# prs-eth/ResDepth

Measured on AMD Instinct MI355X. Metric: DSM tiles/sec fwd+bwd (256x256, 3-ch, depth-5 U-Net), higher is better.
Workload: dtype f32

## Files before the change

### resdepth_amd/csrc/rd_elementwise.hip

```cpp
#include <stdlib.h>

#include "rd_common.h"
#include "rd_mfma_dev.h"

namespace rd {

static inline int grid_cap(long g, int cap) {
    if (g > cap) g = cap;
    if (g < 1) g = 1;
    return (int)g;
}

__device__ __forceinline__ float act_fn(float y, float slope) { return y > 0.f ? y : y * slope; }
__device__ __forceinline__ float act_grad(float y, float slope) { return y > 0.f ? 1.f : slope; }

template <int K>
__device__ __forceinline__ void reduce_rows(double (&vals)[K], double* red, int t, int CQ, int RP, bool active) {
#pragma unroll
    for (int k = 0; k < K; ++k) red[k * 256 + t] = active ? vals[k] : 0.0;
    __syncthreads();
    if (t < CQ) {
#pragma unroll
        for (int k = 0; k < K; ++k) {
            double s = 0.0;
// ... 156 lines not shown
            const float v0 = partial[(long)b * 2 * C + col], v1 = partial[(long)(b + 32) * 2 * C + col];
            const float v2 = partial[(long)(b + 64) * 2 * C + col], v3 = partial[(long)(b + 96) * 2 * C + col];
            sacc += ((double)v0 + (double)v1) + ((double)v2 + (double)v3);
        }
        for (; b < nb; b += 32) sacc += (double)partial[(long)b * 2 * C + col];
    }
    red[t] = sacc;
    __syncthreads();
    if (t == 0 && blockIdx.x == 0 && nbt) *nbt += 1;
    if (t < 4 && c < C) {
        double su = 0.0, sq = 0.0;
#pragma unroll
        for (int sl = 0; sl < 32; ++sl) {
            su += red[sl * 8 + t];
            sq += red[sl * 8 + 4 + t];
        }
        const double m = su / count;
        double var = sq / count - m * m;
        if (var < 0.0) var = 0.0;
        mean[c] = (float)m;
        invstd[c] = (float)(1.0 / sqrt(var + (double)eps));
        if (rmean) rmean[c] = (1.f - momentum) * rmean[c] + momentum * (float)m;
        if (rvar) {
            const double unb = count > 1.0 ? var * count / (count - 1.0) : var;
            rvar[c] = (1.f - momentum) * rvar[c] + momentum * (float)unb;
        }
    }
}

__global__ __launch_bounds__(256) void bn_bwd_stats_finalize_kernel(const float* __restrict__ pa, int ra,
                                                                    const float* __restrict__ pb, int rb, int C,
                                                                    double* __restrict__ sums, float* __restrict__ dgamma,
                                                                    float* __restrict__ dbeta, float* __restrict__ dextra) {
    __shared__ double wred[4][4];
    const int t = threadIdx.x, lane = t & 63, wave = t >> 6, CQ = C >> 2;
    const int sidx = blockIdx.x / CQ, cq = blockIdx.x - sidx * CQ;
    const long col = (long)sidx * C + cq * 4, stride = 4L * C;
    double a0 = 0.0, a1 = 0.0, a2 = 0.0, a3 = 0.0;
    for (int src = 0; src < 2; ++src) {
        const float* part = src ? pb : pa;
        const int nb = src ? rb : ra;
        if (!part) continue;
        int b = t;
        for (; b + 768 < nb; b += 1024) {
            const float4 v0 = *reinterpret_cast<const float4*>(part + (long)b * stride + col);
            const float4 v1 = *reinterpret_cast<const float4*>(part + (long)(b + 256) * stride + col);
            const float4 v2 = *reinterpret_cast<const float4*>(part + (long)(b + 512) * stride + col);
            const float4 v3 = *reinterpret_cast<const float4*>(part + (long)(b + 768) * stride + col);
            a0 += ((double)v0.x + (double)v1.x) + ((double)v2.x + (double)v3.x);
            a1 += ((double)v0.y + (double)v1.y) + ((double)v2.y + (double)v3.y);
            a2 += ((double)v0.z + (double)v1.z) + ((double)v2.z + (double)v3.z);
            a3 += ((double)v0.w + (double)v1.w) + ((double)v2.w + (double)v3.w);
        }
        for (; b < nb; b += 256) {
            const float4 v = *reinterpret_cast<const float4*>(part + (long)b * stride + col);
            a0 += v.x; a1 += v.y; a2 += v.z; a3 += v.w;
        }
    }
#pragma unroll
    for (int o = 1; o < 64; o <<= 1) {
        a0 += __shfl_xor(a0, o);
        a1 += __shfl_xor(a1, o);
        a2 += __shfl_xor(a2, o);
        a3 += __shfl_xor(a3, o);
    }
    if (lane == 0) {
        wred[wave][0] = a0; wred[wave][1] = a1; wred[wave][2] = a2; wred[wave][3] = a3;
    }
    __syncthreads();
    if (t < 4) {
        const double r = ((wred[0][t] + wred[1][t]) + wred[2][t]) + wred[3][t];
        const int c = cq * 4 + t;
        sums[col + t] = r;
        if (sidx == 0 && dbeta) dbeta[c] = (float)r;
        if (sidx == 1 && dgamma) dgamma[c] = (float)r;
        if (sidx == 2 && dextra) dextra[c] = (float)r;
    }
}

__global__ __launch_bounds__(512) void bn_reduce_finalize_quad_kernel(const float* __restrict__ partial, int nb, int C, double count,
                                                                      float eps, float momentum, float* __restrict__ mean,
                                                                      float* __restrict__ invstd, float* __restrict__ rmean,
                                                                      float* __restrict__ rvar, int64_t* nbt) {
    __shared__ double red[512][4];
    const int t = threadIdx.x, kind = t & 1, slice = t >> 1, cq = blockIdx.x;
    const float* base = partial + (long)kind * C + cq * 4;
    const long stride = 2L * C;
    double a0 = 0.0, a1 = 0.0, a2 = 0.0, a3 = 0.0;
    int b = slice;
    for (; b + 7 * 256 < nb; b += 8 * 256) {
        float4 v[8];
#pragma unroll
        for (int k = 0; k < 8; ++k) v[k] = *reinterpret_cast<const float4*>(base + (long)(b + 256 * k) * stride);
#pragma unroll
        for (int k = 0; k < 8; ++k) {
            a0 += v[k].x; a1 += v[k].y; a2 += v[k].z; a3 += v[k].w;
        }
    }
    for (; b < nb; b += 256) {
        const float4 v = *reinterpret_cast<const float4*>(base + (long)b * stride);
        a0 += v.x; a1 += v.y; a2 += v.z; a3 += v.w;
    }
    red[t][0] = a0; red[t][1] = a1; red[t][2] = a2; red[t][3] = a3;
    __syncthreads();
    for (int sl = 128; sl >= 1; sl >>= 1) {
        if (slice < sl) {
#pragma unroll
            for (int k = 0; k < 4; ++k) red[t][k] += red[t + 2 * sl][k];
        }
        __syncthreads();
    }
    if (t == 0 && blockIdx.x == 0 && nbt) *nbt += 1;
    if (t < 4) {
        const int c = cq * 4 + t;
        const double su = red[0][t], sq = red[1][t];
        const double m = su / count;
        double var = sq / count - m * m;
        if (var < 0.0) var = 0.0;
        mean[c] = (float)m;
        invstd[c] = (float)(1.0 / sqrt(var + (double)eps));
        if (rmean) rmean[c] = (1.f - momentum) * rmean[c] + momentum * (float)m;
        if (rvar) {
            const double unb = count > 1.0 ? var * count / (count - 1.0) : var;
            rvar[c] = (1.f - momentum) * rvar[c] + momentum * (float)unb;
        }
    }
}

int bn_reduce_finalize(const float* partial, int nb, int c, double count, float eps, float momentum, float* mean, float* invstd,
                       float* rmean, float* rvar, int64_t* nbt, hipStream_t s) {
    if (c % 4 == 0)
        RD_LAUNCH(bn_reduce_finalize_quad_kernel, dim3(c / 4), dim3(512), 0, s, partial, nb, c, count, eps, momentum, mean,
                           invstd, rmean, rvar, nbt);
    else
        RD_LAUNCH(bn_reduce_finalize_kernel, dim3(cdiv(c, 4)), dim3(256), 0, s, partial, nb, c, count, eps, momentum, mean,
                           invstd, rmean, rvar, nbt);
    RD_LAUNCH_CHECK("bn_reduce_finalize");
    return RD_OK;
}

__global__ void bn_eval_stats_kernel(const float* __restrict__ rmean, const float* __restrict__ rvar, float eps,
                                     float* __restrict__ mean, float* __restrict__ invstd, int C) {
    const int c = blockIdx.x * blockDim.x + threadIdx.x;
    if (c >= C) return;
    mean[c] = rmean[c];
    invstd[c] = 1.f / sqrtf(rvar[c] + eps);
}

template <bool POOL>
__global__ __launch_bounds__(256) void bn_act_pool_fwd_kernel(const float* __restrict__ z, const float* __restrict__ mean,
                                                              const float* __restrict__ invstd,
                                                              const float* __restrict__ gamma,
                                                              const float* __restrict__ beta, float slope_val,
                                                              const float* __restrict__ slope_dev,
                                                              float* __restrict__ a, float* __restrict__ pooled,
                                                              uint8_t* __restrict__ idx, float* __restrict__ zpool, long rows,
                                                              int H, int W, int C, int CQ, unsigned* a_amax, unsigned* p_amax) {
    const float slope = slope_dev ? slope_dev[0] : slope_val;
    const long total = rows * CQ;
    float amx = 0.f, pmx = 0.f;
    long e0, e1;
    block_range(total, blockIdx.x, gridDim.x, blockDim.x, e0, e1);
    for (long e = e0 + threadIdx.x; e < e1; e += blockDim.x) {
        const int cq = (int)(e % CQ);
        const long row = e / CQ;
        const float4 mu = *reinterpret_cast<const float4*>(mean + cq * 4);
        const float4 is = *reinterpret_cast<const float4*>(invstd + cq * 4);
        const float4 ga = *reinterpret_cast<const float4*>(gamma + cq * 4);
        const float4 be = *reinterpret_cast<const float4*>(beta + cq * 4);
        const float sc[4] = {is.x * ga.x, is.y * ga.y, is.z * ga.z, is.w * ga.w};
        const float sh[4] = {be.x - mu.x * sc[0], be.y - mu.y * sc[1], be.z - mu.z * sc[2], be.w - mu.w * sc[3]};
        if (!POOL) {
            const float4 x = ld_nt4(z + row * C + cq * 4);
            float4 y;
            y.x = act_fn(fmaf(x.x, sc[0], sh[0]), slope);
            y.y = act_fn(fmaf(x.y, sc[1], sh[1]), slope);
            y.z = act_fn(fmaf(x.z, sc[2], sh[2]), slope);
            y.w = act_fn(fmaf(x.w, sc[3], sh[3]), slope);
            *reinterpret_cast<float4*>(a + row * C + cq * 4) = y;
            amx = amax_acc(amax_acc(amax_acc(amax_acc(amx, y.x), y.y), y.z), y.w);
        } else {
            const int W2 = W >> 1, H2 = H >> 1;
            const int j = (int)(row % W2);
            const int i = (int)((row / W2) % H2);
            const long img = row / ((long)W2 * H2);
            const long base = (img * H + 2 * i) * W + 2 * j;
            float m[4], zm[4] = {0.f, 0.f, 0.f, 0.f};
            int mi[4] = {0, 0, 0, 0};
#pragma unroll
            for (int k = 0; k < 4; ++k) {
                const long pix = base + (k >> 1) * W + (k & 1);
                const float4 x = ld_nt4(z + pix * C + cq * 4);
                const float xv[4] = {x.x, x.y, x.z, x.w};
                float y[4];
                y[0] = act_fn(fmaf(x.x, sc[0], sh[0]), slope);
                y[1] = act_fn(fmaf(x.y, sc[1], sh[1]), slope);
                y[2] = act_fn(fmaf(x.z, sc[2], sh[2]), slope);
                y[3] = act_fn(fmaf(x.w, sc[3], sh[3]), slope);
                if (a) *reinterpret_cast<float4*>(a + pix * C + cq * 4) = make_float4(y[0], y[1], y[2], y[3]);
#pragma unroll
                for (int q = 0; q < 4; ++q) {
                    if (k == 0 || y[q] > m[q] || y[q] != y[q]) {
                        m[q] = y[q];
                        mi[q] = k;
                        zm[q] = xv[q];
                    }
                }
            }
            *reinterpret_cast<float4*>(pooled + row * C + cq * 4) = make_float4(m[0], m[1], m[2], m[3]);
            pmx = amax_acc(amax_acc(amax_acc(amax_acc(pmx, m[0]), m[1]), m[2]), m[3]);
            if (zpool) st_nt4(zpool + row * C + cq * 4, make_float4(zm[0], zm[1], zm[2], zm[3]));
            st_nt_u8x4(idx + row * C + cq * 4,
                       make_uchar4((unsigned char)mi[0], (unsigned char)mi[1], (unsigned char)mi[2], (unsigned char)mi[3]));
        }
// ... 1153 lines not shown
                       mean, invstd, running_mean, running_var, nbt, c);
    RD_LAUNCH_CHECK("bn_finalize");
    return RD_OK;
}

int rd_bn_eval_stats(const float* running_mean, const float* running_var, float eps, float* mean, float* invstd, int c,
                     rd_stream_t s) {
    RD_REQUIRE(running_mean && running_var && mean && invstd && c > 0, "rd_bn_eval_stats: bad arguments");
    RD_LAUNCH(bn_eval_stats_kernel, dim3(cdiv(c, 256)), dim3(256), 0, (hipStream_t)s, running_mean,
                       running_var, eps, mean, invstd, c);
    RD_LAUNCH_CHECK("bn_eval_stats");
    return RD_OK;
}

int rd_bn_act_pool_fwd(const float* z, const float* mean, const float* invstd, const float* gamma, const float* beta,
                       float slope, const float* slope_dev, float* a, float* pooled, uint8_t* idx, float* zpool, int n, int h,
                       int w, int c, rd_stream_t s) {
    RD_REQUIRE(z && mean && invstd && gamma && beta && (a || pooled), "rd_bn_act_pool_fwd: null pointer");
    RD_REQUIRE(c % 4 == 0 && c > 0, "rd_bn_act_pool_fwd: C must be a multiple of 4 (got %d)", c);
    const QuantArgs qa = quant_take();
    const int CQ = c / 4;
    const long pixels = (long)n * h * w;
    if (pooled) {
        RD_REQUIRE(idx && h % 2 == 0 && w % 2 == 0, "rd_bn_act_pool_fwd: pooling needs idx and even H, W");
        const long rows = pixels / 4;
        ProfScope ps((hipStream_t)s, "bn_act_pool_fwd", 0,
                     4.0 * pixels * c * (a ? 2.25 : 1.25) + 0.25 * pixels * c + (zpool ? 1.0 * pixels * c : 0.0));
        RD_LAUNCH((bn_act_pool_fwd_kernel<true>), dim3(grid_cap((rows * CQ + 255) / 256, 8192)), dim3(256), 0,
                           (hipStream_t)s, z, mean, invstd, gamma, beta, slope, slope_dev, a, pooled, idx, zpool, rows, h, w, c,
                           CQ, (unsigned*)nullptr, qa.out2);
    } else {
        ProfScope ps((hipStream_t)s, "bn_act_fwd", 0, 8.0 * pixels * c);
        RD_LAUNCH((bn_act_pool_fwd_kernel<false>), dim3(grid_cap((pixels * CQ + 255) / 256, 8192)), dim3(256),
                           0, (hipStream_t)s, z, mean, invstd, gamma, beta, slope, slope_dev, a, (float*)nullptr,
                           (uint8_t*)nullptr, (float*)nullptr, pixels, h, w, c, CQ, qa.out, (unsigned*)nullptr);
    }
    RD_LAUNCH_CHECK("bn_act_pool_fwd");
    return RD_OK;
}

size_t rd_bn_act_bwd_ws_bytes(int n, int h, int w, int c) {
    RowPlan pl;
    if (!plan_rows((long)n * h * w, c, &pl)) return 0;
    return (size_t)pl.nb * 4 * c * sizeof(double);
}

int rd_bn_act_bwd_reduce(const float* z, const float* mean, const float* invstd, const float* gamma, const float* beta,
                         float slope, const float* slope_dev, const float* g_full, const float* g_pool,
                         const uint8_t* idx, double* sums, float* dgamma, float* dbeta, float* dextra, int n, int h, int w, int c,
                         void* ws, size_t ws_bytes, rd_stream_t s) {
    RD_REQUIRE(z && mean && invstd && gamma && beta && sums, "rd_bn_act_bwd_reduce: null pointer");
    RD_REQUIRE(g_full || g_pool, "rd_bn_act_bwd_reduce: no gradient source");
    RD_REQUIRE(!g_pool || idx, "rd_bn_act_bwd_reduce: g_pool needs idx");
    const bool pool = g_pool != nullptr;
    const long pixels = (long)n * h * w;
    const long rows = pool ? pixels / 4 : pixels;
    RowPlan pl;
    RD_REQUIRE(plan_rows(rows, c, &pl), "rd_bn_act_bwd_reduce: C must be a multiple of 4 and <= 1024 (got %d)", c);
    size_t need = (size_t)pl.nb * 4 * c * sizeof(double);
    if (const size_t q = rd_bn_act_bwd_ws_bytes(n, h, w, c); q > need) need = q;
    if (!ws || ws_bytes < need) {
        set_error("rd_bn_act_bwd_reduce: workspace too small (%zu < %zu)", ws_bytes, need);
        return RD_ERR_WS;
    }
    ProfScope ps((hipStream_t)s, "bn_act_bwd_reduce", 0, 4.0 * pixels * c * (1 + (g_full ? 1 : 0) + (pool ? 0.3 : 0)));
    if (pool)
        RD_LAUNCH((bn_act_bwd_kernel<true, false>), dim3(pl.nb), dim3(256), 0, (hipStream_t)s, z, mean, invstd,
                           gamma, beta, slope, slope_dev, g_full, g_pool, idx, (double*)ws, (const double*)nullptr, 1.0, 1,
                           (float*)nullptr, rows, h, w, c, pl.CQ, pl.RP, pl.rows_per_block, (unsigned*)nullptr);
    else
        RD_LAUNCH((bn_act_bwd_kernel<false, false>), dim3(pl.nb), dim3(256), 0, (hipStream_t)s, z, mean,
                           invstd, gamma, beta, slope, slope_dev, g_full, g_pool, idx, (double*)ws, (const double*)nullptr, 1.0, 1,
                           (float*)nullptr, rows, h, w, c, pl.CQ, pl.RP, pl.rows_per_block, (unsigned*)nullptr);
    RD_LAUNCH(partial_reduce_kernel, dim3(cdiv(4 * c, 16)), dim3(256), 0, (hipStream_t)s, (const double*)ws,
                       sums, pl.nb, 4 * c, c, dbeta, dgamma, dextra);
    RD_LAUNCH_CHECK("bn_act_bwd_reduce");
    return RD_OK;
}

int rd_bn_bwd_stats_finalize(const float* part_a, int rows_a, const float* part_b, int rows_b, int c, double* sums,
                             float* dgamma, float* dbeta, float* dextra, rd_stream_t s) {
    RD_REQUIRE(part_a && rows_a > 0 && sums && c > 0 && c % 4 == 0 && (!part_b || rows_b > 0), "rd_bn_bwd_stats_finalize: bad arguments");
    ProfScope ps((hipStream_t)s, "bn_act_bwd_reduce", 0, 16.0 * c * ((double)rows_a + (part_b ? rows_b : 0)));
    RD_LAUNCH(bn_bwd_stats_finalize_kernel, dim3(c), dim3(256), 0, (hipStream_t)s, part_a, rows_a, part_b,
                       part_b ? rows_b : 0, c, sums, dgamma, dbeta, dextra);
    RD_LAUNCH_CHECK("bn_bwd_stats_finalize");
    return RD_OK;
}

int rd_bn_act_bwd_apply(const float* z, const float* mean, const float* invstd, const float* gamma, const float* beta,
                        float slope, const float* slope_dev, const float* g_full, const float* g_pool,
                        const uint8_t* idx, const double* sums,
                        double count, int training, float* dz, float* dgamma, float* dbeta, int n, int h, int w, int c,
                        rd_stream_t s) {
    RD_REQUIRE(z && mean && invstd && gamma && beta && sums && dz, "rd_bn_act_bwd_apply: null pointer");
    RD_REQUIRE(g_full || g_pool, "rd_bn_act_bwd_apply: no gradient source");
    RD_REQUIRE(!g_pool || idx, "rd_bn_act_bwd_apply: g_pool needs idx");
    RD_REQUIRE(count > 0, "rd_bn_act_bwd_apply: count must be positive");
    const QuantArgs qa = quant_take();
    const bool pool = g_pool != nullptr;
    const long pixels = (long)n * h * w;
    const long rows = pool ? pixels / 4 : pixels;
    RowPlan pl;
    RD_REQUIRE(plan_rows(rows, c, &pl), "rd_bn_act_bwd_apply: C must be a multiple of 4 and <= 1024 (got %d)", c);
    {
        ProfScope ps((hipStream_t)s, "bn_act_bwd_apply", 0,
                     4.0 * pixels * c * (2 + (g_full ? 1 : 0) + (pool ? 0.3 : 0)));
        if (pool)
            RD_LAUNCH((bn_act_bwd_kernel<true, true>), dim3(pl.nb), dim3(256), 0, (hipStream_t)s, z, mean,
                               invstd, gamma, beta, slope, slope_dev, g_full, g_pool, idx, (double*)nullptr, sums, count,
                               training, dz, rows, h, w, c, pl.CQ, pl.RP, pl.rows_per_block, qa.out);
        else
            RD_LAUNCH((bn_act_bwd_kernel<false, true>), dim3(pl.nb), dim3(256), 0, (hipStream_t)s, z, mean,
                               invstd, gamma, beta, slope, slope_dev, g_full, g_pool, idx, (double*)nullptr, sums, count, training,
                               dz, rows, h, w, c, pl.CQ, pl.RP, pl.rows_per_block, qa.out);
    }
    if (dgamma || dbeta)
        RD_LAUNCH(bn_param_grad_kernel, dim3(cdiv(c, 256)), dim3(256), 0, (hipStream_t)s, sums, dgamma, dbeta,
                           c);
    RD_LAUNCH_CHECK("bn_act_bwd_apply");
    return RD_OK;
}

}

static int first_grid(int n, int h, int w, int* tiles_x, int* tiles_y, int* ntiles) {
    *tiles_x = cdiv(w, FT_W);
    *tiles_y = cdiv(h, FT_H);
    *ntiles = n * (*tiles_x) * (*tiles_y);
    return *ntiles < 512 ? *ntiles : 512;
}

template <bool WGRAD>
static int launch_first(const float* x, const float* wt, float* z, const float* dz, float* partial, int n, int h, int w,
                        int cin, int cout, int grid, int tiles_x, int tiles_y, int ntiles, hipStream_t s) {
    const int CQ = cout / 4, PS = 256 / CQ;
#define RD_FIRST_CASE(CI)                                                                                              \
    case CI:                                                                                                           \
        RD_LAUNCH((conv_first_kernel<CI, WGRAD>), dim3(grid), dim3(256), 0, s, x, wt, z, dz, partial, n, h, w, \
                           cout, CQ, PS, tiles_x, tiles_y, ntiles);                                                    \
        break;
    switch (cin) {
        RD_FIRST_CASE(1)
        RD_FIRST_CASE(2)
        RD_FIRST_CASE(3)
        RD_FIRST_CASE(4)
        RD_FIRST_CASE(5)
        RD_FIRST_CASE(6)
        default:
            set_error("first conv supports 1..6 input channels (got %d)", cin);
            return RD_ERR_ARG;
    }
#undef RD_FIRST_CASE
    return RD_OK;
}

extern "C" {

int rd_conv3x3_first_fwd(const float* x, const float* wt, float* z, int n, int h, int w, int cin, int cout,
                         rd_stream_t s) {
    return rd_conv3x3_first_fwd_stats(x, wt, z, nullptr, n, h, w, cin, cout, nullptr, 0, s);
}

int rd_conv3x3_first_fwd_act_available(int n, int h, int w, int cin, int cout) {
    return conv_first_seg_tiles(n, h, w, cin, cout) > 0 && h % 2 == 0 && w % 2 == 0;
}

int rd_conv3x3_first_fwd_act(const float* x, const float* wt, const float* mean, const float* invstd, const float* gamma,
// ... 632 lines not shown
```

### resdepth_amd/csrc/rd_igemm.hip

```cpp
#include <stdlib.h>
#include <string.h>

#include <type_traits>

#include "rd_common.h"
#include "rd_mfma_dev.h"
#include "rd_nt.h"

namespace rd {

template <int BM, int BN, int WM, int WN, int AMODE, int EPI>
__global__ __launch_bounds__(256) void igemm_nt_kernel(NtParams p) {
    constexpr int BK = 32, LS = BK + 4;
    constexpr int TM = BM / WM / 32, TN = BN / WN / 32;
    constexpr int AI = BM / 32, BI = BN / 32;
    __shared__ __attribute__((aligned(16))) float smem[(BM + BN) * LS];
    float* As = smem;
    float* Bs = smem + BM * LS;

    const int lb = xcd_remap(blockIdx.x, gridDim.x);
    const int tile_n = lb % p.tiles_n, tile_m = lb / p.tiles_n;
    const int m0 = tile_m * BM, n0 = tile_n * BN;
    const int t = threadIdx.x, lane = t & 63, wave = t >> 6;
    const int wm = wave / WN, wn = wave % WN;
// ... 1311 lines not shown
__global__ __launch_bounds__(256) void wgrad_tn_split_kernel(TnParams p) {
    __shared__ __attribute__((aligned(16))) float smem[2 * (BM + BN) * 32];
    const Quant qz = quant_select(p.a_amax, p.b_amax);
    if (qz.use3) wgrad_tn_split_body<3, BM, BN, WM, WN, AMODE, BMODE>(p, smem, qz);
    else wgrad_tn_split_body<6, BM, BN, WM, WN, AMODE, BMODE>(p, smem, qz);
}

struct TnPlan {
    int bm, bn, tiles_m, tiles_n, splits, kchunk;
};

static TnPlan plan_tn(int M, int N, long Kp) {
    TnPlan pl;
    pl.bm = M > 64 ? 128 : 64;
    pl.bn = N > 64 ? 128 : 64;
    const int tforce = tune(TUNE_TN_TILE);
    if (tforce > 0) {
        pl.bm = tforce / 1000;
        pl.bn = tforce % 1000;
    }
    pl.tiles_m = cdiv(M, pl.bm);
    pl.tiles_n = cdiv(N, pl.bn);
    const int tiles = pl.tiles_m * pl.tiles_n;
    long ktiles = (Kp + 31) / 32;
    const int target = tune(TUNE_TN_BLOCKS);
    long want = target / tiles;
    if (want < 1) want = 1;
    long maxs = ktiles / 8 > 0 ? ktiles / 8 : 1;
    long s = want < maxs ? want : maxs;
    if (s < 1) s = 1;
    if (s > 512) s = 512;
    long per = (ktiles + s - 1) / s;
    pl.kchunk = (int)(per * 32);
    pl.splits = (int)((ktiles + per - 1) / per);
    return pl;
}

template <int AMODE, int BMODE>
static int launch_tn(TnParams p, const TnPlan& pl, hipStream_t s, const char* cls) {
    char pcls[64];
    const int tn_force = tune(TUNE_TN_SPLIT);
    const int split = tn_force >= 0 ? tn_force : (mfma_split() && pl.bm == 128 && pl.bn == 128);
    snprintf(pcls, sizeof(pcls), "%s|wgrad_tn%s<%d,%d,%d,%d>", cls, split ? "_split" : "", pl.bm, pl.bn, AMODE, BMODE);
    ProfScope ps(s, pcls, 2.0 * p.M * p.N * (double)p.Kp,
                 4.0 * ((double)p.Kp * p.lda * (AMODE == WA_UP2 ? 4 : 1) + (double)p.Kp * p.ldb + (double)p.M * p.N), true);
    const double a_bytes = 4.0 * (double)p.Kp * p.lda * (AMODE == WA_UP2 ? 4 : 1), b_bytes = 4.0 * (double)p.Kp * p.ldb;
    if (a_bytes >= 4294967040.0 || b_bytes >= 4294967040.0) {
        set_error("%s: operand larger than the 4 GiB buffer-descriptor range", cls);
        return RD_ERR_ARG;
    }
    p.a_bytes = (unsigned)a_bytes;
    p.b_bytes = (unsigned)b_bytes;
    p.kchunk = pl.kchunk;
    p.tiles_n = pl.tiles_n;
    p.tiles_mn = pl.tiles_m * pl.tiles_n;
    if (!split || mfma_products() != 3 || !p.a_amax || !p.b_amax) p.a_amax = p.b_amax = nullptr;
    const int grid = p.tiles_mn * pl.splits;
    if (split) {
        if (pl.bm == 128 && pl.bn == 128)
            RD_LAUNCH((wgrad_tn_split_kernel<128, 128, 2, 2, AMODE, BMODE>), dim3(grid), dim3(256), 0, s, p);
        else if (pl.bm == 128)
            RD_LAUNCH((wgrad_tn_split_kernel<128, 64, 2, 2, AMODE, BMODE>), dim3(grid), dim3(256), 0, s, p);
        else if (pl.bn == 128)
            RD_LAUNCH((wgrad_tn_split_kernel<64, 128, 2, 2, AMODE, BMODE>), dim3(grid), dim3(256), 0, s, p);
        else
            RD_LAUNCH((wgrad_tn_split_kernel<64, 64, 2, 2, AMODE, BMODE>), dim3(grid), dim3(256), 0, s, p);
        RD_LAUNCH_CHECK(cls);
        return RD_OK;
    }
    if (pl.bm == 128 && pl.bn == 128)
        RD_LAUNCH((wgrad_tn_kernel<128, 128, 2, 2, AMODE, BMODE>), dim3(grid), dim3(256), 0, s, p);
    else if (pl.bm == 128)
        RD_LAUNCH((wgrad_tn_kernel<128, 64, 2, 2, AMODE, BMODE>), dim3(grid), dim3(256), 0, s, p);
    else if (pl.bn == 128)
        RD_LAUNCH((wgrad_tn_kernel<64, 128, 2, 2, AMODE, BMODE>), dim3(grid), dim3(256), 0, s, p);
    else
        RD_LAUNCH((wgrad_tn_kernel<64, 64, 2, 2, AMODE, BMODE>), dim3(grid), dim3(256), 0, s, p);
    RD_LAUNCH_CHECK(cls);
    return RD_OK;
}

template <int SPT>
__global__ __launch_bounds__(256) void slab_reduce_kernel(const float* __restrict__ slab, float* __restrict__ dw, int M,
                                                          int N, int splits, int mode, int Cin, int Cout) {
    const long total = (long)M * N, quads = total >> 2;
    const long nthreads = (long)gridDim.x * blockDim.x;
    for (long gid = (long)blockIdx.x * blockDim.x + threadIdx.x; gid < quads * SPT; gid += nthreads) {
        const long q = gid / SPT;
        const int part = (int)(gid - q * SPT);
        const float4* src = reinterpret_cast<const float4*>(slab) + q;
        double a0 = 0.0, a1 = 0.0, a2 = 0.0, a3 = 0.0;
        int s = part;
        for (; s + 3 * SPT < splits; s += 4 * SPT) {
            const float4 v0 = src[(long)s * quads], v1 = src[(long)(s + SPT) * quads];
            const float4 v2 = src[(long)(s + 2 * SPT) * quads], v3 = src[(long)(s + 3 * SPT) * quads];
            a0 += ((double)v0.x + (double)v1.x) + ((double)v2.x + (double)v3.x);
            a1 += ((double)v0.y + (double)v1.y) + ((double)v2.y + (double)v3.y);
            a2 += ((double)v0.z + (double)v1.z) + ((double)v2.z + (double)v3.z);
            a3 += ((double)v0.w + (double)v1.w) + ((double)v2.w + (double)v3.w);
        }
        for (; s < splits; s += SPT) {
            const float4 v = src[(long)s * quads];
            a0 += v.x; a1 += v.y; a2 += v.z; a3 += v.w;
        }
#pragma unroll
        for (int o = 1; o < SPT; o <<= 1) {
            a0 += __shfl_xor(a0, o);
            a1 += __shfl_xor(a1, o);
            a2 += __shfl_xor(a2, o);
            a3 += __shfl_xor(a3, o);
        }
        if (part != 0) continue;
        const long e = q << 2;
        const int m = (int)(e / N), n = (int)(e - (long)m * N);
        const float r[4] = {(float)a0, (float)a1, (float)a2, (float)a3};
        if (mode == 3) {
            const int tq = n / Cout, co = n - tq * Cout;
#pragma unroll
            for (int k = 0; k < 4; ++k) dw[((long)(co + k) * Cin + m) * 9 + (8 - tq)] = r[k];
        } else if (mode == 2) {
            *reinterpret_cast<float4*>(dw + e) = make_float4(r[0], r[1], r[2], r[3]);
        } else if (mode == 0) {
            const int tap = n / Cin, ci = n - tap * Cin;
#pragma unroll
            for (int k = 0; k < 4; ++k) dw[((long)m * Cin + ci + k) * 9 + tap] = r[k];
        } else {
            const int ab = m / Cout, co = m - ab * Cout;
#pragma unroll
            for (int k = 0; k < 4; ++k) dw[((long)(n + k) * Cout + co) * 4 + ab] = r[k];
        }
    }
}

static void launch_slab_reduce(const float* slab, float* dw, int M, int N, int splits, int mode, int Cin, int Cout, hipStream_t s) {
#if RD_DIAG_SLAB_READ_DIV
    splits = (splits + RD_DIAG_SLAB_READ_DIV - 1) / RD_DIAG_SLAB_READ_DIV;
#endif
    const long quads = (long)M * N / 4;
    int spt = 1;
    while (spt < 16 && quads * spt < 262144 && 2 * spt <= splits) spt *= 2;
    const int grid = grid_for(quads * spt, 256, 4096);
    if (spt == 1) RD_LAUNCH(slab_reduce_kernel<1>, dim3(grid), dim3(256), 0, s, slab, dw, M, N, splits, mode, Cin, Cout);
    else if (spt == 2) RD_LAUNCH(slab_reduce_kernel<2>, dim3(grid), dim3(256), 0, s, slab, dw, M, N, splits, mode, Cin, Cout);
    else if (spt == 4) RD_LAUNCH(slab_reduce_kernel<4>, dim3(grid), dim3(256), 0, s, slab, dw, M, N, splits, mode, Cin, Cout);
    else if (spt == 8) RD_LAUNCH(slab_reduce_kernel<8>, dim3(grid), dim3(256), 0, s, slab, dw, M, N, splits, mode, Cin, Cout);
    else RD_LAUNCH(slab_reduce_kernel<16>, dim3(grid), dim3(256), 0, s, slab, dw, M, N, splits, mode, Cin, Cout);
}

__global__ void pack_conv3x3_kernel(const float* __restrict__ w, float* __restrict__ wf, float* __restrict__ wd,
                                    int cout, int cin) {
    const long total = (long)cout * cin * 9;
    for (long e = (long)blockIdx.x * blockDim.x + threadIdx.x; e < total; e += (long)gridDim.x * blockDim.x) {
        const int ci = (int)(e % cin);
        const int tap = (int)((e / cin) % 9);
        const int co = (int)(e / ((long)cin * 9));
        wf[e] = w[((long)co * cin + ci) * 9 + tap];
        if (wd) {
            const int co2 = (int)(e % cout);
            const int tap2 = (int)((e / cout) % 9);
            const int ci2 = (int)(e / ((long)cout * 9));
            wd[e] = w[((long)co2 * cin + ci2) * 9 + (8 - tap2)];
        }
    }
}

__global__ __launch_bounds__(256) void tiled_transpose_kernel(const float* __restrict__ in, float* __restrict__ out, int rows,
                                                              int groups, int cols, int flip) {
    __shared__ float tile[32][33];
    const int tiles_c = (cols + 31) / 32, tiles_r = (rows + 31) / 32;
    const int tx = threadIdx.x & 31, ty = threadIdx.x >> 5;
    for (long b = blockIdx.x; b < (long)groups * tiles_r * tiles_c; b += gridDim.x) {
        const int tc = (int)(b % tiles_c), tr = (int)((b / tiles_c) % tiles_r), g = (int)(b / ((long)tiles_c * tiles_r));
        const int r0 = tr * 32, c0 = tc * 32;
#pragma unroll
        for (int k = 0; k < 4; ++k) {
            const int r = r0 + ty + 8 * k, c = c0 + tx;
            tile[ty + 8 * k][tx] = (r < rows && c < cols) ? in[((long)r * groups + g) * cols + c] : 0.f;
        }
        __syncthreads();
        const int go = flip ? groups - 1 - g : g;
#pragma unroll
        for (int k = 0; k < 4; ++k) {
            const int c = c0 + ty + 8 * k, r = r0 + tx;
            if (r < rows && c < cols) out[((long)c * groups + go) * rows + r] = tile[tx][ty + 8 * k];
        }
        __syncthreads();
    }
}


__global__ void pack_convt_kernel(const float* __restrict__ w, float* __restrict__ wtf, float* __restrict__ wtd,
                                  int cin, int cout) {
    const long total = (long)cin * cout * 4;
    for (long e = (long)blockIdx.x * blockDim.x + threadIdx.x; e < total; e += (long)gridDim.x * blockDim.x) {
        const int ci = (int)(e % cin);
        const int co = (int)((e / cin) % cout);
        const int ab = (int)(e / ((long)cin * cout));
        wtf[e] = w[((long)ci * cout + co) * 4 + ab];
        if (wtd) {
            const int co2 = (int)(e % cout);
            const int ab2 = (int)((e / cout) % 4);
            const int ci2 = (int)(e / ((long)cout * 4));
            wtd[e] = w[((long)ci2 * cout + co2) * 4 + ab2];
        }
    }
}

static int grid_for(long total, int block = 256, int cap = 4096) {
    long g = (total + block - 1) / block;
    if (g > cap) g = cap;
    if (g < 1) g = 1;
    return (int)g;
}

static int check_conv_args(int n, int h, int w, int cin, int cout) {
    RD_REQUIRE(n > 0 && h > 0 && w > 0 && cin > 0 && cout > 0, "bad conv shape n=%d h=%d w=%d cin=%d cout=%d", n, h, w,
               cin, cout);
    RD_REQUIRE((long)n * h * w * 4L < (1L << 31), "pixel count too large for 32-bit tile indices");
    return RD_OK;
}

}

using namespace rd;

extern "C" {

int rd_mfma_products(void) { return mfma_products(); }

// ... 475 lines not shown
```

Baseline: 4564.

## Parallelize BN stat finalization across block groups and tile weight-gradient slab reduction

```diff
diff --git a/resdepth_amd/csrc/rd_elementwise.hip b/resdepth_amd/csrc/rd_elementwise.hip
--- a/resdepth_amd/csrc/rd_elementwise.hip
+++ b/resdepth_amd/csrc/rd_elementwise.hip
@@ -262,7 +262,7 @@
                                                                       float eps, float momentum, float* __restrict__ mean,
                                                                       float* __restrict__ invstd, float* __restrict__ rmean,
                                                                       float* __restrict__ rvar, int64_t* nbt) {
-    __shared__ double red[512][4];
+    __shared__ double red[4][512], red2[4][128], fin[2][4];
     const int t = threadIdx.x, kind = t & 1, slice = t >> 1, cq = blockIdx.x;
     const float* base = partial + (long)kind * C + cq * 4;
     const long stride = 2L * C;
@@ -281,19 +281,32 @@
         const float4 v = *reinterpret_cast<const float4*>(base + (long)b * stride);
         a0 += v.x; a1 += v.y; a2 += v.z; a3 += v.w;
     }
-    red[t][0] = a0; red[t][1] = a1; red[t][2] = a2; red[t][3] = a3;
+    red[0][t] = a0; red[1][t] = a1; red[2][t] = a2; red[3][t] = a3;
     __syncthreads();
-    for (int sl = 128; sl >= 1; sl >>= 1) {
-        if (slice < sl) {
-#pragma unroll
-            for (int k = 0; k < 4; ++k) red[t][k] += red[t + 2 * sl][k];
-        }
-        __syncthreads();
-    }
+    if (t < 128) {
+#pragma unroll
+        for (int k = 0; k < 4; ++k) red2[k][t] = (red[k][t] + red[k][t + 256]) + (red[k][t + 128] + red[k][t + 384]);
+    }
+    __syncthreads();
+    if (t < 64) {
+        double r[4];
+#pragma unroll
+        for (int k = 0; k < 4; ++k) r[k] = red2[k][t] + red2[k][t + 64];
+#pragma unroll
+        for (int o = 32; o >= 2; o >>= 1) {
+#pragma unroll
+            for (int k = 0; k < 4; ++k) r[k] += __shfl_xor(r[k], o);
+        }
+        if (t < 2) {
+#pragma unroll
+            for (int k = 0; k < 4; ++k) fin[t][k] = r[k];
+        }
+    }
+    __syncthreads();
     if (t == 0 && blockIdx.x == 0 && nbt) *nbt += 1;
     if (t < 4) {
         const int c = cq * 4 + t;
-        const double su = red[0][t], sq = red[1][t];
+        const double su = fin[0][t], sq = fin[1][t];
         const double m = su / count;
         double var = sq / count - m * m;
         if (var < 0.0) var = 0.0;
@@ -307,9 +320,217 @@
     }
 }
 
+constexpr int kCoopRows = 2048;
+constexpr int kCoopBlocksPerGroup = 16;
+
+__device__ __forceinline__ void coop_publish(double* grp_scratch, int cl, int slice, double a0, double a1, double a2, double a3) {
+    double* o = grp_scratch + ((long)cl * 256 + slice) * 4;
+    __hip_atomic_store(o + 0, a0, __ATOMIC_RELAXED, __HIP_MEMORY_SCOPE_AGENT);
+    __hip_atomic_store(o + 1, a1, __ATOMIC_RELAXED, __HIP_MEMORY_SCOPE_AGENT);
+    __hip_atomic_store(o + 2, a2, __ATOMIC_RELAXED, __HIP_MEMORY_SCOPE_AGENT);
+    __hip_atomic_store(o + 3, a3, __ATOMIC_RELAXED, __HIP_MEMORY_SCOPE_AGENT);
+}
+
+__device__ __forceinline__ bool coop_arrive(unsigned* ticket, int* flag) {
+    __atomic_signal_fence(__ATOMIC_SEQ_CST);
+    asm volatile("s_waitcnt vmcnt(0)" ::: "memory");
+    __syncthreads();
+    if (threadIdx.x == 0) {
+        const unsigned prev = __hip_atomic_fetch_add(ticket, 1u, __ATOMIC_RELAXED, __HIP_MEMORY_SCOPE_AGENT);
+        *flag = prev == (unsigned)(kCoopBlocksPerGroup - 1);
+        if (*flag) __hip_atomic_store(ticket, 0u, __ATOMIC_RELAXED, __HIP_MEMORY_SCOPE_AGENT);
+    }
+    __syncthreads();
+    const bool last = *flag != 0;
+    __atomic_signal_fence(__ATOMIC_SEQ_CST);
+    return last;
+}
+
+__device__ __forceinline__ double coop_load(const double* p) {
+    return __hip_atomic_load(p, __ATOMIC_RELAXED, __HIP_MEMORY_SCOPE_AGENT);
+}
+
+__global__ __launch_bounds__(256) void bn_reduce_finalize_coop_kernel(const float* __restrict__ partial, int nb, int C, double count,
+                                                                     float eps, float momentum, float* __restrict__ mean,
+                                                                     float* __restrict__ invstd, float* __restrict__ rmean,
+                                                                     float* __restrict__ rvar, int64_t* nbt,
+                                                                     double* scratch, unsigned* tickets) {
+    __shared__ int flag;
+    __shared__ double tot[16][4];
+    const int t = threadIdx.x, grp = blockIdx.x / kCoopBlocksPerGroup, blk = blockIdx.x - grp * kCoopBlocksPerGroup;
+    const int cl = t & 15, slice = blk * 16 + (t >> 4);
+    const float* base = partial + (long)(cl >> 3) * C + (grp * 8 + (cl & 7)) * 4;
+    const long stride = 2L * C;
+    double* gs = scratch + (long)grp * (16 * 256 * 4);
+    double a0 = 0.0, a1 = 0.0, a2 = 0.0, a3 = 0.0;
+    int b = slice;
+    for (; b + 31 * 256 < nb; b += 32 * 256) {
+        float4 v[32];
+#pragma unroll
+        for (int k = 0; k < 32; ++k) v[k] = *reinterpret_cast<const float4*>(base + (long)(b + 256 * k) * stride);
+#pragma unroll
+        for (int k = 0; k < 32; ++k) {
+            a0 += v[k].x; a1 += v[k].y; a2 += v[k].z; a3 += v[k].w;
+        }
+    }
+    for (; b + 7 * 256 < nb; b += 8 * 256) {
+        float4 v[8];
+#pragma unroll
+        for (int k = 0; k < 8; ++k) v[k] = *reinterpret_cast<const float4*>(base + (long)(b + 256 * k) * stride);
+#pragma unroll
+        for (int k = 0; k < 8; ++k) {
+            a0 += v[k].x; a1 += v[k].y; a2 += v[k].z; a3 += v[k].w;
+        }
+    }
+    for (; b < nb; b += 256) {
+        const float4 v = *reinterpret_cast<const float4*>(base + (long)b * stride);
+        a0 += v.x; a1 += v.y; a2 += v.z; a3 += v.w;
+    }
+    coop_publish(gs, cl, slice, a0, a1, a2, a3);
+    if (!coop_arrive(tickets + grp, &flag)) return;
+    const int j = t & 15;
+    {
+        const int col = t >> 4;
+        const double* src = gs + ((long)col * 256 + j) * 4;
+        double r[4];
+#pragma unroll
+        for (int k = 0; k < 4; ++k) {
+            double x[16];
+#pragma unroll
+            for (int m = 0; m < 16; ++m) x[m] = coop_load(src + (long)m * 64 + k);
+            const double y0 = (x[0] + x[8]) + (x[4] + x[12]);
+            const double y1 = (x[2] + x[10]) + (x[6] + x[14]);
+            const double y2 = (x[1] + x[9]) + (x[5] + x[13]);
+            const double y3 = (x[3] + x[11]) + (x[7] + x[15]);
+            r[k] = (y0 + y1) + (y2 + y3);
+        }
+#pragma unroll
+        for (int o = 8; o >= 1; o >>= 1) {
+#pragma unroll
+            for (int k = 0; k < 4; ++k) r[k] += __shfl_xor(r[k], o);
+        }
+        if (j == 0) {
+#pragma unroll
+            for (int k = 0; k < 4; ++k) tot[col][k] = r[k];
+        }
+    }
+    __syncthreads();
+    if (t == 0 && grp == 0 && nbt) *nbt += 1;
+    if (t < 32) {
+        const int q = t >> 2, k = t & 3, c = (grp * 8 + q) * 4 + k;
+        const double su = tot[q][k], sq = tot[8 + q][k];
+        const double m = su / count;
+        double var = sq / count - m * m;
+        if (var < 0.0) var = 0.0;
+        mean[c] = (float)m;
+        invstd[c] = (float)(1.0 / sqrt(var + (double)eps));
+        if (rmean) rmean[c] = (1.f - momentum) * rmean[c] + momentum * (float)m;
+        if (rvar) {
+            const double unb = count > 1.0 ? var * count / (count - 1.0) : var;
+            rvar[c] = (1.f - momentum) * rvar[c] + momentum * (float)unb;
+        }
+    }
+}
+
+__global__ __launch_bounds__(256) void bn_bwd_stats_finalize_coop_kernel(const float* __restrict__ pa, int ra,
+                                                                        const float* __restrict__ pb, int rb, int C,
+                                                                        double* __restrict__ sums, float* __restrict__ dgamma,
+                                                                        float* __restrict__ dbeta, float* __restrict__ dextra,
+                                                                        double* scratch, unsigned* tickets) {
+    __shared__ int flag;
+    const int t = threadIdx.x, grp = blockIdx.x / kCoopBlocksPerGroup, blk = blockIdx.x - grp * kCoopBlocksPerGroup;
+    const int cl = t & 15, slice = blk * 16 + (t >> 4);
+    const long col0 = (long)(grp * 16 + cl) * 4, stride = 4L * C;
+    double* gs = scratch + (long)grp * (16 * 256 * 4);
+    double a0 = 0.0, a1 = 0.0, a2 = 0.0, a3 = 0.0;
+    for (int src = 0; src < 2; ++src) {
+        const float* part = src ? pb : pa;
+        const int nb = src ? rb : ra;
+        if (!part) continue;
+        int b = slice;
+        for (; b + 15 * 256 < nb; b += 16 * 256) {
+            float4 v[16];
+#pragma unroll
+            for (int k = 0; k < 16; ++k) v[k] = *reinterpret_cast<const float4*>(part + (long)(b + 256 * k) * stride + col0);
+#pragma unroll
+            for (int k = 0; k < 16; k += 4) {
+                a0 += ((double)v[k].x + (double)v[k + 1].x) + ((double)v[k + 2].x + (double)v[k + 3].x);
+                a1 += ((double)v[k].y + (double)v[k + 1].y) + ((double)v[k + 2].y + (double)v[k + 3].y);
+                a2 += ((double)v[k].z + (double)v[k + 1].z) + ((double)v[k + 2].z + (double)v[k + 3].z);
+                a3 += ((double)v[k].w + (double)v[k + 1].w) + ((double)v[k + 2].w + (double)v[k + 3].w);
+            }
+        }
+        for (; b + 768 < nb; b += 1024) {
+            const float4 v0 = *reinterpret_cast<const float4*>(part + (long)b * stride + col0);
+            const float4 v1 = *reinterpret_cast<const float4*>(part + (long)(b + 256) * stride + col0);
+            const float4 v2 = *reinterpret_cast<const float4*>(part + (long)(b + 512) * stride + col0);
+            const float4 v3 = *reinterpret_cast<const float4*>(part + (long)(b + 768) * stride + col0);
+            a0 += ((double)v0.x + (double)v1.x) + ((double)v2.x + (double)v3.x);
+            a1 += ((double)v0.y + (double)v1.y) + ((double)v2.y + (double)v3.y);
+            a2 += ((double)v0.z + (double)v1.z) + ((double)v2.z + (double)v3.z);
+            a3 += ((double)v0.w + (double)v1.w) + ((double)v2.w + (double)v3.w);
+        }
+        for (; b < nb; b += 256) {
+            const float4 v = *reinterpret_cast<const float4*>(part + (long)b * stride + col0);
+            a0 += v.x; a1 += v.y; a2 += v.z; a3 += v.w;
+        }
+    }
+    coop_publish(gs, cl, slice, a0, a1, a2, a3);
+    if (!coop_arrive(tickets + grp, &flag)) return;
+    const int j = t & 15;
+    {
+        const int col = t >> 4;
+        const double* src = gs + ((long)col * 256 + j * 16) * 4;
+        double r[4];
+#pragma unroll
+        for (int k = 0; k < 4; ++k) {
+            double x[16];
+#pragma unroll
+            for (int m = 0; m < 16; ++m) x[m] = coop_load(src + m * 4 + k);
+            const double y0 = (x[0] + x[1]) + (x[2] + x[3]), y1 = (x[4] + x[5]) + (x[6] + x[7]);
+            const double y2 = (x[8] + x[9]) + (x[10] + x[11]), y3 = (x[12] + x[13]) + (x[14] + x[15]);
+            r[k] = (y0 + y1) + (y2 + y3);
+        }
+#pragma unroll
+        for (int o = 1; o <= 2; o <<= 1) {
+#pragma unroll
+            for (int k = 0; k < 4; ++k) r[k] += __shfl_xor(r[k], o);
+        }
+#pragma unroll
+        for (int k = 0; k < 4; ++k) {
+            const double w0 = __shfl(r[k], 0, 16), w1 = __shfl(r[k], 4, 16), w2 = __shfl(r[k], 8, 16), w3 = __shfl(r[k], 12, 16);
+            r[k] = ((w0 + w1) + w2) + w3;
+        }
+        if (j < 4) {
+            const long column = (long)(grp * 16 + col) * 4 + j;
+            const double v = j == 0 ? r[0] : j == 1 ? r[1] : j == 2 ? r[2] : r[3];
+            const int sidx = (int)(column / C), c = (int)(column - (long)sidx * C);
+            sums[column] = v;
+            if (sidx == 0 && dbeta) dbeta[c] = (float)v;
+            if (sidx == 1 && dgamma) dgamma[c] = (float)v;
+            if (sidx == 2 && dextra) dextra[c] = (float)v;
+        }
+    }
+}
+
+static bool coop_scratch(hipStream_t s, int groups, double** scratch, unsigned** tickets) {
+    float* slab = nullptr;
+    size_t slab_bytes = 0;
+    int n_tickets = 0;
+    if (!splitk_workspace(s, tickets, &n_tickets, &slab, &slab_bytes)) return false;
+    if (groups > n_tickets || (size_t)groups * (16 * 256 * 4) * sizeof(double) > slab_bytes) return false;
+    *scratch = reinterpret_cast<double*>(slab);
+    return true;
+}
+
 int bn_reduce_finalize(const float* partial, int nb, int c, double count, float eps, float momentum, float* mean, float* invstd,
                        float* rmean, float* rvar, int64_t* nbt, hipStream_t s) {
-    if (c % 4 == 0)
+    double* scratch = nullptr;
+    unsigned* tickets = nullptr;
+    if (c % 32 == 0 && nb >= kCoopRows && coop_scratch(s, c / 32, &scratch, &tickets))
+        RD_LAUNCH(bn_reduce_finalize_coop_kernel, dim3(c / 32 * kCoopBlocksPerGroup), dim3(256), 0, s, partial, nb, c, count, eps,
+                           momentum, mean, invstd, rmean, rvar, nbt, scratch, tickets);
+    else if (c % 4 == 0)
         RD_LAUNCH(bn_reduce_finalize_quad_kernel, dim3(c / 4), dim3(512), 0, s, partial, nb, c, count, eps, momentum, mean,
                            invstd, rmean, rvar, nbt);
     else
@@ -1629,8 +1850,14 @@
                              float* dgamma, float* dbeta, float* dextra, rd_stream_t s) {
     RD_REQUIRE(part_a && rows_a > 0 && sums && c > 0 && c % 4 == 0 && (!part_b || rows_b > 0), "rd_bn_bwd_stats_finalize: bad arguments");
     ProfScope ps((hipStream_t)s, "bn_act_bwd_reduce", 0, 16.0 * c * ((double)rows_a + (part_b ? rows_b : 0)));
-    RD_LAUNCH(bn_bwd_stats_finalize_kernel, dim3(c), dim3(256), 0, (hipStream_t)s, part_a, rows_a, part_b,
-                       part_b ? rows_b : 0, c, sums, dgamma, dbeta, dextra);
+    double* scratch = nullptr;
+    unsigned* tickets = nullptr;
+    if (c % 32 == 0 && (long)rows_a + (part_b ? rows_b : 0) >= kCoopRows && coop_scratch((hipStream_t)s, c / 16, &scratch, &tickets))
+        RD_LAUNCH(bn_bwd_stats_finalize_coop_kernel, dim3(c / 16 * kCoopBlocksPerGroup), dim3(256), 0, (hipStream_t)s, part_a,
+                           rows_a, part_b, part_b ? rows_b : 0, c, sums, dgamma, dbeta, dextra, scratch, tickets);
+    else
+        RD_LAUNCH(bn_bwd_stats_finalize_kernel, dim3(c), dim3(256), 0, (hipStream_t)s, part_a, rows_a, part_b,
+                           part_b ? rows_b : 0, c, sums, dgamma, dbeta, dextra);
     RD_LAUNCH_CHECK("bn_bwd_stats_finalize");
     return RD_OK;
 }
diff --git a/resdepth_amd/csrc/rd_igemm.hip b/resdepth_amd/csrc/rd_igemm.hip
--- a/resdepth_amd/csrc/rd_igemm.hip
+++ b/resdepth_amd/csrc/rd_igemm.hip
@@ -1417,15 +1417,55 @@
 
 template <int SPT>
 __global__ __launch_bounds__(256) void slab_reduce_kernel(const float* __restrict__ slab, float* __restrict__ dw, int M,
-                                                          int N, int splits, int mode, int Cin, int Cout) {
-    const long total = (long)M * N, quads = total >> 2;
-    const long nthreads = (long)gridDim.x * blockDim.x;
-    for (long gid = (long)blockIdx.x * blockDim.x + threadIdx.x; gid < quads * SPT; gid += nthreads) {
-        const long q = gid / SPT;
-        const int part = (int)(gid - q * SPT);
-        const float4* src = reinterpret_cast<const float4*>(slab) + q;
+                                                          int N, int splits, int mode, int Cin, int Cout, int RT) {
+    extern __shared__ float stile[];
+    const long quads = ((long)M * N) >> 2;
+    const int t = threadIdx.x;
+    const int nrow = mode == 1 ? Cout : M;
+    const int ncol = mode == 3 ? Cout : Cin;
+    const int G = mode == 2 ? 1 : (mode == 1 ? 4 : 9);
+    const int ncs = (ncol + 31) >> 5;
+    const int rt = blockIdx.x / ncs, cs = blockIdx.x - rt * ncs;
+    const int r0 = rt * RT, rows = min(RT, nrow - r0);
+    const int c0 = cs << 5, cw = min(32, ncol - c0), cw4 = cw >> 2;
+    int SR, SC, LS, L, nruns;
+    long dst0, dstride;
+    if (mode == 0) {
+        L = cw * 9; LS = L; nruns = rows; SR = LS; SC = 9;
+        dst0 = ((long)r0 * Cin + c0) * 9; dstride = (long)Cin * 9;
+    } else if (mode == 3) {
+        L = rows * 9; LS = RT * 9 + 1; nruns = cw; SR = 9; SC = LS;
+        dst0 = ((long)c0 * Cin + r0) * 9; dstride = (long)Cin * 9;
+    } else if (mode == 1) {
+        L = rows * 4; LS = RT * 4 + 1; nruns = cw; SR = 4; SC = LS;
+        dst0 = ((long)c0 * Cout + r0) * 4; dstride = (long)Cout * 4;
+    } else {
+        L = cw; LS = 33; nruns = rows; SR = LS; SC = 1;
+        dst0 = (long)r0 * N + c0; dstride = N;
+    }
+    const int per_row = G * cw4, ntask = rows * per_row * SPT;
+    for (int i = t; i < ntask; i += 256) {
+        const int q = i / SPT, part = i - q * SPT;
+        const int r = q / per_row, rem = q - r * per_row;
+        const int g = rem / cw4, cq = rem - g * cw4;
+        long e;
+        if (mode == 1) e = ((long)g * Cout + r0 + r) * N + c0 + cq * 4;
+        else e = (long)(r0 + r) * N + (long)g * ncol + c0 + cq * 4;
+        const float4* src = reinterpret_cast<const float4*>(slab) + (e >> 2);
         double a0 = 0.0, a1 = 0.0, a2 = 0.0, a3 = 0.0;
         int s = part;
+        for (; s + 7 * SPT < splits; s += 8 * SPT) {
+            float4 v[8];
+#pragma unroll
+            for (int k = 0; k < 8; ++k) v[k] = src[(long)(s + k * SPT) * quads];
+#pragma unroll
+            for (int k = 0; k < 8; k += 4) {
+                a0 += ((double)v[k].x + (double)v[k + 1].x) + ((double)v[k + 2].x + (double)v[k + 3].x);
+                a1 += ((double)v[k].y + (double)v[k + 1].y) + ((double)v[k + 2].y + (double)v[k + 3].y);
+                a2 += ((double)v[k].z + (double)v[k + 1].z) + ((double)v[k + 2].z + (double)v[k + 3].z);
+                a3 += ((double)v[k].w + (double)v[k + 1].w) + ((double)v[k + 2].w + (double)v[k + 3].w);
+            }
+        }
         for (; s + 3 * SPT < splits; s += 4 * SPT) {
             const float4 v0 = src[(long)s * quads], v1 = src[(long)(s + SPT) * quads];
             const float4 v2 = src[(long)(s + 2 * SPT) * quads], v3 = src[(long)(s + 3 * SPT) * quads];
@@ -1446,23 +1486,22 @@
             a3 += __shfl_xor(a3, o);
         }
         if (part != 0) continue;
-        const long e = q << 2;
-        const int m = (int)(e / N), n = (int)(e - (long)m * N);
-        const float r[4] = {(float)a0, (float)a1, (float)a2, (float)a3};
-        if (mode == 3) {
-            const int tq = n / Cout, co = n - tq * Cout;
-#pragma unroll
-            for (int k = 0; k < 4; ++k) dw[((long)(co + k) * Cin + m) * 9 + (8 - tq)] = r[k];
-        } else if (mode == 2) {
-            *reinterpret_cast<float4*>(dw + e) = make_float4(r[0], r[1], r[2], r[3]);
-        } else if (mode == 0) {
-            const int tap = n / Cin, ci = n - tap * Cin;
-#pragma unroll
-            for (int k = 0; k < 4; ++k) dw[((long)m * Cin + ci + k) * 9 + tap] = r[k];
+        float* o = stile + r * SR + (cq * 4) * SC + (mode == 3 ? 8 - g : g);
+        o[0] = (float)a0; o[SC] = (float)a1; o[2 * SC] = (float)a2; o[3 * SC] = (float)a3;
+    }
+    __syncthreads();
+    const int ppr = ((L + 3) >> 2) + 1;
+    for (int i = t; i < nruns * ppr; i += 256) {
+        const int j = i / ppr, p = i - j * ppr;
+        float* d = dw + dst0 + (long)j * dstride;
+        const float* sl = stile + j * LS;
+        const int h = min((int)((0 - (reinterpret_cast<uintptr_t>(d) >> 2)) & 3), L);
+        const int b = p == 0 ? 0 : h + (p - 1) * 4;
+        const int en = p == 0 ? h : min(b + 4, L);
+        if (p != 0 && en - b == 4) {
+            *reinterpret_cast<float4*>(d + b) = make_float4(sl[b], sl[b + 1], sl[b + 2], sl[b + 3]);
         } else {
-            const int ab = m / Cout, co = m - ab * Cout;
-#pragma unroll
-            for (int k = 0; k < 4; ++k) dw[((long)(n + k) * Cout + co) * 4 + ab] = r[k];
+            for (int x = b; x < en; ++x) d[x] = sl[x];
         }
     }
 }
@@ -1474,12 +1513,16 @@
     const long quads = (long)M * N / 4;
     int spt = 1;
     while (spt < 16 && quads * spt < 262144 && 2 * spt <= splits) spt *= 2;
-    const int grid = grid_for(quads * spt, 256, 4096);
-    if (spt == 1) RD_LAUNCH(slab_reduce_kernel<1>, dim3(grid), dim3(256), 0, s, slab, dw, M, N, splits, mode, Cin, Cout);
-    else if (spt == 2) RD_LAUNCH(slab_reduce_kernel<2>, dim3(grid), dim3(256), 0, s, slab, dw, M, N, splits, mode, Cin, Cout);
-    else if (spt == 4) RD_LAUNCH(slab_reduce_kernel<4>, dim3(grid), dim3(256), 0, s, slab, dw, M, N, splits, mode, Cin, Cout);
-    else if (spt == 8) RD_LAUNCH(slab_reduce_kernel<8>, dim3(grid), dim3(256), 0, s, slab, dw, M, N, splits, mode, Cin, Cout);
-    else RD_LAUNCH(slab_reduce_kernel<16>, dim3(grid), dim3(256), 0, s, slab, dw, M, N, splits, mode, Cin, Cout);
+    const int rt = cdiv(mode == 1 ? 32 : 16, spt);
+    const int nrow = mode == 1 ? Cout : M, ncol = mode == 3 ? Cout : Cin;
+    const int grid = cdiv(nrow, rt) * cdiv(ncol, 32);
+    const int lds_floats = mode == 0 ? rt * 288 : mode == 3 ? 32 * (rt * 9 + 1) : mode == 1 ? 32 * (rt * 4 + 1) : rt * 33;
+    const size_t lds = (size_t)lds_floats * sizeof(float);
+    if (spt == 1) RD_LAUNCH(slab_reduce_kernel<1>, dim3(grid), dim3(256), lds, s, slab, dw, M, N, splits, mode, Cin, Cout, rt);
+    else if (spt == 2) RD_LAUNCH(slab_reduce_kernel<2>, dim3(grid), dim3(256), lds, s, slab, dw, M, N, splits, mode, Cin, Cout, rt);
+    else if (spt == 4) RD_LAUNCH(slab_reduce_kernel<4>, dim3(grid), dim3(256), lds, s, slab, dw, M, N, splits, mode, Cin, Cout, rt);
+    else if (spt == 8) RD_LAUNCH(slab_reduce_kernel<8>, dim3(grid), dim3(256), lds, s, slab, dw, M, N, splits, mode, Cin, Cout, rt);
+    else RD_LAUNCH(slab_reduce_kernel<16>, dim3(grid), dim3(256), lds, s, slab, dw, M, N, splits, mode, Cin, Cout, rt);
 }
 
 __global__ void pack_conv3x3_kernel(const float* __restrict__ w, float* __restrict__ wf, float* __restrict__ wd,
```

Result: no change. 4570, median of 6 (+0.1%).
